# haoyu94/RoITr

Hardware: AMD Instinct MI355X
Metric: point-cloud pairs/s (higher is better)
Workload: dtype f32

## Files before the change

include/roitr_engine.h:

```cpp
#ifndef ROITR_ENGINE_H
#define ROITR_ENGINE_H

#include <stddef.h>

#ifdef __cplusplus
extern "C" {
#endif

#ifndef ROITR_POINTOPS_H
typedef struct ihipStream_t* roitr_stream_t;
#endif

typedef struct RoitrGemm {
    int M, N, K;
    const float* A; const float* A2; int lda; const int* a_idx; int a_limit;
    const float* W; int ldw; const int* w_idx; int w_limit;
    const float* bias; float alpha; int relu;
    float* C; int ldc;
    int batch; long sA, sW, sC, sBias, sAidx, sWidx;
    const int* seg_off; int seg_a0, seg_w0;
    const float* ln_gamma; const float* ln_beta; const float* ln_res; const int* ln_res_idx; const float* ln_post;
    int ln_relu; float ln_eps;
    int bf16;
    const float* A_cat; int lda_cat; int k_cat;
    const float* ip_feat; const int* ip_idx; const float* ip_dist2;
    const int* a_cat_idx;
    const int* batch_live;
    long w_piece;
} RoitrGemm;
#define ROITR_BF16_W 1
#define ROITR_BF16_A 2
#define ROITR_BF16_C 4
#define ROITR_BF16_X3 8
int roitr_gemm(const RoitrGemm* g, roitr_stream_t stream);
int roitr_gemm_bf16_supported(const RoitrGemm* g);
int roitr_f32_to_bf16(long n, const float* src, unsigned short* dst, roitr_stream_t stream);
int roitr_gemm_x3_supported(const RoitrGemm* g);
int roitr_split_bf16x3(long n, const float* src, unsigned short* dst, long piece, roitr_stream_t stream);

int roitr_add_layernorm(int M, int C, const float* x, const float* res, const int* res_idx, const float* gamma,
                        const float* beta, const float* post_add, int relu, float eps, float* out, roitr_stream_t stream);
int roitr_add_layernorm_interp(int M, int C, const float* x, const float* res, const int* res_idx, const float* gamma,
                               const float* beta, int relu, float eps, const float* ip_feat, const int* ip_idx, const float* ip_dist2,
                               float* out, roitr_stream_t stream);
int roitr_l2_normalize(int M, int C, const float* x, float* out, roitr_stream_t stream);
int roitr_transpose(int rows, int cols, const float* in, int ld_in, float* out, int ld_out, roitr_stream_t stream);
int roitr_add_vectors(int n, const float* a, const float* b, float* out, roitr_stream_t stream);
int roitr_interp3_add(int n, int C, const float* feat, const int* idx, const float* dist2, const float* base, float* out,
                      roitr_stream_t stream);
int roitr_segment_mean(int b, int C, const float* x, const int* offset, float* out, roitr_stream_t stream);
int roitr_sinusoid(long rows, int C, const float* vals, const float* div_term, float* out, roitr_stream_t stream);
int roitr_geo_embed(long rows, int C, int angle_k, const float* d_idx, const float* a_idx, const float* div_term,
                    const float* Wd, const float* bd, const float* Wa, const float* ba, float* out, roitr_stream_t stream);
int roitr_split3_bf16(long n, const float* src, unsigned short* dst, roitr_stream_t stream);
int roitr_geo_embed_split(long rows, int C, int angle_k, const float* d_idx, const float* a_idx, const float* div_term,
                          const unsigned short* Wd3, const float* bd, const unsigned short* Wa3, const float* ba, float* out,
                          roitr_stream_t stream);
int roitr_geo_embed_bf16(long rows, int C, int angle_k, const float* d_idx, const float* a_idx, const float* div_term,
                         const unsigned short* Wd, const float* bd, const unsigned short* Wa, const float* ba, float* out,
                         roitr_stream_t stream);
int roitr_geo_embed_bf16_out(long rows, int C, int angle_k, const float* d_idx, const float* a_idx, const float* div_term,
                             const unsigned short* Wd, const float* bd, const unsigned short* Wa, const float* ba,
                             unsigned short* out, roitr_stream_t stream);
size_t roitr_geo_table_floats(int C, int n_int_d, int n_int_a);
int roitr_geo_table_build(int C, const float* div_term, const float* Wd, const float* bd, const float* Wa, const float* ba,
                          float interval, int n_int_d, int n_int_a, float* table, double* fit);
int roitr_geo_embed_table(long rows, int C, int angle_k, const float* d_idx, const float* a_idx, const float* table, float interval,
                          int n_int_d, int n_int_a, const float* div_term, const float* Wd, const float* bd, const float* Wa,
                          const float* ba, void* out, int out_bf16, roitr_stream_t stream);
int roitr_geo_combine(long rows, int C, int k, const float* pd, const float* pa, float* out, roitr_stream_t stream);
int roitr_gather_rows(long rows, int C, const float* in, const int* idx, int limit, float* out, roitr_stream_t stream);
int roitr_compose_idx(int n, const int* outer, const int* inner, int* out, roitr_stream_t stream);
int roitr_calc_ppf(int m, int k, const float* centre_xyz, const float* centre_normals, const float* ref_xyz,
                   const float* ref_normals, const int* group_idx, float* out, roitr_stream_t stream);

typedef struct RoitrLocalAttn {
    int M, K, H, heads;
    const float* q; int ldq;
    const float* k; int ldk;
    const float* v; int ldv;
    const int* group_idx; const float* ppf;
    const float* wvpe; const float* bvpe;
    float scale;
    float* out; int ldo;
    const void* node_order;
    int bf16;
    const float* wpe; const float* bpe;
} RoitrLocalAttn;
int roitr_local_attention(const RoitrLocalAttn* a, roitr_stream_t stream);
int roitr_build_pfold(int H, int heads, const float* wpe, const float* bpe, float* pfold, roitr_stream_t stream);

typedef struct RoitrLocalAttnFold {
    int M, in_dim, H;
    const float* x; int ldx;
    const float* q; int ldq;
    const float* qt;
    const int* group_idx; const float* ppf;
    const float* wpe;
    const float* wvpe; const float* bvpe;
    float scale;
    float* xbar;
    float* vpart;
    const void* node_order;
    int ldqt;
} RoitrLocalAttnFold;
int roitr_local_attention_fold(const RoitrLocalAttnFold* a, roitr_stream_t stream);
int roitr_local_attention_fold_supported(int in_dim, int H, int K);

typedef struct RoitrLocalBlock {
    int M, K, H;
    const float* x; const float* kv; const int* group_idx; const float* ppf;
    const void* node_order;
    const float* wq; const float* bq;
    const float* wpe; const float* bpe; const float* wvpe; const float* bvpe;
    const float* wcat; const float* bcat; const float* norm_w; const float* norm_b;
    const float* wout; const float* bout; const float* bn2_w; const float* bn2_b;
    float scale, eps;
    float* out;
    int kv_bf16;
    const unsigned short* wq_h; const unsigned short* wcat_h; const unsigned short* wout_h;
} RoitrLocalBlock;
int roitr_local_block(const RoitrLocalBlock* a, roitr_stream_t stream);
int roitr_local_block_supported(int H, int K);

typedef struct RoitrLocalTd {
    int M, in_dim, H;
    const float* x; const int* node_idx;
    const int* group_idx; const float* ppf;
    const void* node_order;
    const float* wqqt; const float* bqqt;
    const float* wv; const float* bv;
    const float* wpe; const float* wvpe; const float* bvpe;
    const float* wcat; const float* bcat; const float* norm_w; const float* norm_b;
    const float* wout; const float* bout;
    float scale, eps;
    float* out;
} RoitrLocalTd;
int roitr_local_td(const RoitrLocalTd* a, roitr_stream_t stream);
int roitr_local_td_supported(int in_dim, int H, int K);

typedef struct RoitrLocalFirst {
    int M, K;
    const float* x; const int* group_idx; const float* ppf; const void* node_order;
    const float* head_consts; const float* G; const float* zero_bias;
    const float* norm_w; const float* norm_b; const float* wout; const float* bout;
    float scale, eps;
    float* out;
} RoitrLocalFirst;
int roitr_local_first(const RoitrLocalFirst* a, roitr_stream_t stream);

int roitr_geo_indices(int rows, const float* pts, const int* offset, const int* cloud_of_row, const long* eoff,
                      float sigma_d, float sigma_a, int angle_k, int n_max, float* d_idx, float* a_idx, roitr_stream_t stream);
// ... 189 lines not shown
```

roitr_amd/_lib.py:

```python
import ctypes
import os

_HERE = os.path.dirname(os.path.abspath(__file__))
LIB_PATH = os.path.join(_HERE, "lib", "libroitr_hip.so")
_lib = None


class RoitrError(RuntimeError):
    pass


def lib():
    global _lib
    if _lib is None:
        if not os.path.exists(LIB_PATH):
            raise RoitrError(
                f"{LIB_PATH} is missing: build it with `python -m roitr_amd.build` "
                "(hipcc --offload-arch=gfx950).  roitr_amd has no CPU fallback.")
        import torch
        _lib = ctypes.CDLL(LIB_PATH)
        _lib.roitr_last_error.restype = ctypes.c_char_p
        _lib.roitr_knn_workspace_bytes.restype = ctypes.c_size_t
        _lib.roitr_geo_table_floats.restype = ctypes.c_size_t
        for name in ("roitr_engine_create",):
            if hasattr(_lib, name):
                getattr(_lib, name).restype = ctypes.c_void_p
    return _lib


def check(status, what=""):
    if status != 0:
        raise RoitrError(f"{what} failed with status {status}: {lib().roitr_last_error().decode()}")


def ptr(t):
    if t is None:
        return ctypes.c_void_p(0)
    if not t.is_cuda:
        raise RoitrError("roitr_amd needs ROCm device tensors (no CPU fallback): got a tensor on " + str(t.device))
    return ctypes.c_void_p(t.data_ptr())


def host_ptr(t):
    if t.is_cuda:
        raise RoitrError("host_ptr: expected a CPU tensor")
    return ctypes.c_void_p(t.data_ptr())


def stream_ptr():
    import torch
    return ctypes.c_void_p(torch.cuda.current_stream().cuda_stream)


def c_float(x):
    return ctypes.c_float(float(x))
```

roitr_amd/csrc/geo_table.hip:

```cpp
#include "common.h"
#include <mutex>
#include "prof.h"
#include <cmath>
#include <vector>

namespace {

constexpr int NCOEF = 8, CS = 64;

__device__ __forceinline__ void sincos_cw(float x, float& sn, float& cs)
{
    const float k = rintf(x * 0.63661977236758134f);
    float r = fmaf(-k, 1.57079637050628662109375f, x);
    r = fmaf(-k, -4.37113900018624283e-8f, r);
    r = fmaf(-k, -1.71512449944201e-15f, r);
    const float z = r * r;
    float ps = fmaf(fmaf(-1.9515295891e-4f, z, 8.3321608736e-3f), z, -1.6666654611e-1f);
    ps = fmaf(ps * z, r, r);
    float pc = fmaf(fmaf(2.443315711809948e-5f, z, -1.388731625493765e-3f), z, 4.166664568298827e-2f);
    pc = fmaf(pc * z, z, fmaf(-0.5f, z, 1.0f));
    const int q = (int)k;
    const float s1 = (q & 1) ? pc : ps, c1 = (q & 1) ? ps : pc;
    sn = (q & 2) ? -s1 : s1;
    cs = ((q + 1) & 2) ? -c1 : c1;
}

__device__ __noinline__ float geo_direct(float x, const float* __restrict__ W, const float* __restrict__ bias,
                                         const float* __restrict__ div, int C, int col)
{
    const float* w = W + (size_t)col * C;
    float acc = 0.f;
    for (int i = 0; i < C / 2; ++i) {
        float sn, cs;
        sincos_cw(x * div[i], sn, cs);
        acc = fmaf(sn, w[2 * i], acc);
        acc = fmaf(cs, w[2 * i + 1], acc);
    }
    return acc + bias[col];
}

__device__ __forceinline__ float poly8(const float4* __restrict__ p, float t)
{
    const float4 lo = p[0], hi = p[CS];
    float a = fmaf(hi.w, t, hi.z);
    a = fmaf(a, t, hi.y);
    a = fmaf(a, t, hi.x);
    a = fmaf(a, t, lo.w);
    a = fmaf(a, t, lo.z);
    a = fmaf(a, t, lo.y);
    return fmaf(a, t, lo.x);
}

__device__ __forceinline__ void locate(float x, float inv_h, int n, int base, int& j, float& t)
{
    const float u = x * inv_h;
    const float fl = floorf(u);
    const bool ok = u >= 0.f && fl < (float)n;
    j = ok ? base + (int)fl : -1;
    t = fmaf(2.f, u - fl, -1.f);
}

struct GeoTableArgs {
    long rows;
    int C, nd, na;
    float inv_h;
    const float *d_idx, *a_idx, *table, *div, *Wd, *bd, *Wa, *ba;
    void* out;
};

template <bool OH>
__device__ __forceinline__ void geo_table_body(const GeoTableArgs& g)
{
    extern __shared__ __attribute__((aligned(16))) float tab[];
    const int tid = threadIdx.x, lane = tid & 63, wave = tid >> 6, nwaves = blockDim.x >> 6;
    const int slice = blockIdx.x, nint = g.nd + g.na;
    {
        const float4* src = reinterpret_cast<const float4*>(g.table + (size_t)slice * nint * (NCOEF * CS));
        float4* dst = reinterpret_cast<float4*>(tab);
        for (int i = tid; i < nint * (NCOEF * CS / 4); i += blockDim.x) dst[i] = src[i];
    }
    __syncthreads();
    const int col = slice * CS + lane;
    const float4* tl = reinterpret_cast<const float4*>(tab) + lane;
    const long nchunks = (g.rows + 63) >> 6;
    for (long q = (long)blockIdx.y * nwaves + wave; q < nchunks; q += (long)gridDim.y * nwaves) {
        const long row0 = q << 6, row = row0 + lane;
        float xd = 0.f, xa0 = 0.f, xa1 = 0.f, xa2 = 0.f;
        if (row < g.rows) {
            xd = g.d_idx[row];
            xa0 = g.a_idx[row * 3]; xa1 = g.a_idx[row * 3 + 1]; xa2 = g.a_idx[row * 3 + 2];
        }
        int jd, j0, j1, j2; float td, t0, t1, t2;
        locate(xd, g.inv_h, g.nd, 0, jd, td);
        locate(xa0, g.inv_h, g.na, g.nd, j0, t0);
        locate(xa1, g.inv_h, g.na, g.nd, j1, t1);
        locate(xa2, g.inv_h, g.na, g.nd, j2, t2);
        const int cnt = (int)min(64L, g.rows - row0);
#pragma unroll 2
        for (int e = 0; e < cnt; ++e) {
            const int sjd = __builtin_amdgcn_readlane(jd, e), sj0 = __builtin_amdgcn_readlane(j0, e);
            const int sj1 = __builtin_amdgcn_readlane(j1, e), sj2 = __builtin_amdgcn_readlane(j2, e);
            const float std_ = __uint_as_float(__builtin_amdgcn_readlane(__float_as_uint(td), e));
            const float st0 = __uint_as_float(__builtin_amdgcn_readlane(__float_as_uint(t0), e));
            const float st1 = __uint_as_float(__builtin_amdgcn_readlane(__float_as_uint(t1), e));
            const float st2 = __uint_as_float(__builtin_amdgcn_readlane(__float_as_uint(t2), e));
            float vd, v0, v1, v2;
            if (__builtin_expect((sjd | sj0 | sj1 | sj2) >= 0, 1)) {
                vd = poly8(tl + sjd * (2 * CS), std_);
                v0 = poly8(tl + sj0 * (2 * CS), st0);
                v1 = poly8(tl + sj1 * (2 * CS), st1);
                v2 = poly8(tl + sj2 * (2 * CS), st2);
            } else {
                const float sxd = __uint_as_float(__builtin_amdgcn_readlane(__float_as_uint(xd), e));
                const float sx0 = __uint_as_float(__builtin_amdgcn_readlane(__float_as_uint(xa0), e));
                const float sx1 = __uint_as_float(__builtin_amdgcn_readlane(__float_as_uint(xa1), e));
                const float sx2 = __uint_as_float(__builtin_amdgcn_readlane(__float_as_uint(xa2), e));
                vd = sjd >= 0 ? poly8(tl + sjd * (2 * CS), std_) : geo_direct(sxd, g.Wd, g.bd, g.div, g.C, col);
                v0 = sj0 >= 0 ? poly8(tl + sj0 * (2 * CS), st0) : geo_direct(sx0, g.Wa, g.ba, g.div, g.C, col);
                v1 = sj1 >= 0 ? poly8(tl + sj1 * (2 * CS), st1) : geo_direct(sx1, g.Wa, g.ba, g.div, g.C, col);
                v2 = sj2 >= 0 ? poly8(tl + sj2 * (2 * CS), st2) : geo_direct(sx2, g.Wa, g.ba, g.div, g.C, col);
            }
            const float val = vd + fmaxf(v0, fmaxf(v1, v2));
            const size_t o = (size_t)(row0 + e) * g.C + col;
            if (OH) {
                typedef __bf16 bf16x2_t __attribute__((ext_vector_type(2)));
                typedef float f32x2_t __attribute__((ext_vector_type(2)));
                const float vo = __int_as_float(__builtin_amdgcn_update_dpp(0, __float_as_int(val), 0xB1, 0xf, 0xf, true));
                f32x2_t pr = {val, vo};
                if ((threadIdx.x & 1) == 0)
                    *reinterpret_cast<unsigned*>(reinterpret_cast<unsigned short*>(g.out) + o) = __builtin_bit_cast(unsigned, __builtin_convertvector(pr, bf16x2_t));
            } else reinterpret_cast<float*>(g.out)[o] = val;
        }
    }
}

__global__ __launch_bounds__(1024) void geo_table_kernel(GeoTableArgs g) { geo_table_body<false>(g); }
__global__ __launch_bounds__(1024) void geo_table_bf16o_kernel(GeoTableArgs g) { geo_table_body<true>(g); }

void exact_rows(double x, const std::vector<double>& div, const float* W, const float* b, int C, std::vector<double>& emb, double* out)
{
    for (int i = 0; i < C / 2; ++i) { emb[2 * i] = sin(x * div[i]); emb[2 * i + 1] = cos(x * div[i]); }
    for (int c = 0; c < C; ++c) {
        const float* w = W + (size_t)c * C;
        double s = 0.0;
        for (int k = 0; k < C; ++k) s += (double)w[k] * emb[k];
        out[c] = s + (double)b[c];
    }
}

}

extern "C" size_t roitr_geo_table_floats(int C, int n_int_d, int n_int_a)
{
    return (size_t)(C / CS) * (size_t)(n_int_d + n_int_a) * NCOEF * CS;
}

extern "C" int roitr_geo_table_build(int C, const float* div_term, const float* Wd, const float* bd, const float* Wa, const float* ba,
                                     float interval, int n_int_d, int n_int_a, float* table, double* fit)
{
    if (C % CS || C <= 0 || n_int_d < 1 || n_int_a < 1 || !(interval > 0.f)) return ROITR_ERR_ARG;
    {
        int ex; if (frexpf(interval, &ex) != 0.5f) return ROITR_ERR_ARG;
    }
    const double h = interval;
    std::vector<double> div(C / 2), emb(C);
    for (int i = 0; i < C / 2; ++i) div[i] = (double)div_term[i];
    double node[NCOEF], tm[NCOEF][NCOEF] = {};
    for (int k = 0; k < NCOEF; ++k) node[k] = cos(M_PI * (2 * k + 1) / (2.0 * NCOEF));
    tm[0][0] = 1.0; tm[1][1] = 1.0;
    for (int m = 2; m < NCOEF; ++m)
        for (int p = 0; p < NCOEF; ++p) tm[m][p] = (p > 0 ? 2.0 * tm[m - 1][p - 1] : 0.0) - tm[m - 2][p];
    constexpr int NPROBE = 64;
    std::vector<double> f((size_t)NCOEF * C), mono((size_t)NCOEF * C), ref(C);
    std::vector<double> err_c[2] = {std::vector<double>(C, 0.0), std::vector<double>(C, 0.0)};
    std::vector<double> amp_c[2] = {std::vector<double>(C, 0.0), std::vector<double>(C, 0.0)};
    const int nint = n_int_d + n_int_a;
    for (int q = 0; q < 6; ++q) fit[q] = 0.0;
    for (int J = 0; J < nint; ++J) {
        const bool dist = J < n_int_d;
        const float* W = dist ? Wd : Wa; const float* b = dist ? bd : ba;
        const double x0 = ((dist ? J : J - n_int_d) + 0.5) * h;
        for (int k = 0; k < NCOEF; ++k) exact_rows(x0 + 0.5 * h * node[k], div, W, b, C, emb, &f[(size_t)k * C]);
        for (int c = 0; c < C; ++c) {
            double a[NCOEF];
            for (int m = 0; m < NCOEF; ++m) {
                double s = 0.0;
                for (int k = 0; k < NCOEF; ++k) s += f[(size_t)k * C + c] * cos(M_PI * m * (2 * k + 1) / (2.0 * NCOEF));
                a[m] = s * (m == 0 ? 1.0 : 2.0) / NCOEF;
            }
            for (int p = 0; p < NCOEF; ++p) {
                double s = 0.0;
                for (int m = p; m < NCOEF; ++m) s += a[m] * tm[m][p];
                mono[(size_t)p * C + c] = s;
                table[((((size_t)(c / CS) * nint + J) * 2 + p / 4) * CS + (c % CS)) * 4 + (p % 4)] = (float)s;
            }
        }
        for (int pi = 0; pi < NPROBE; ++pi) {
            const double t = -1.0 + 2.0 * pi / (double)(NPROBE - 1);
            exact_rows(x0 + 0.5 * h * t, div, W, b, C, emb, ref.data());
            for (int c = 0; c < C; ++c) {
                double v = mono[(size_t)(NCOEF - 1) * C + c];
                for (int p = NCOEF - 2; p >= 0; --p) v = v * t + mono[(size_t)p * C + c];
                double& e = fit[dist ? 0 : 2]; double& amp = fit[dist ? 1 : 3];
                const double d = fabs(v - ref[c]);
                e = fmax(e, d); amp = fmax(amp, fabs(ref[c]));
                err_c[dist ? 0 : 1][c] = fmax(err_c[dist ? 0 : 1][c], d);
                amp_c[dist ? 0 : 1][c] = fmax(amp_c[dist ? 0 : 1][c], fabs(ref[c]));
            }
        }
    }
    for (int q = 0; q < 2; ++q) {
        const double floor_ = fit[q ? 3 : 1] / 1024.0;
        for (int c = 0; c < C; ++c) {
            const double a_ = fmax(amp_c[q][c], floor_);
            if (a_ > 0.0) fit[4 + q] = fmax(fit[4 + q], err_c[q][c] / a_);
        }
    }
    return ROITR_OK;
}

extern "C" int roitr_geo_embed_table(long rows, int C, int angle_k, const float* d_idx, const float* a_idx, const float* table,
                                     float interval, int n_int_d, int n_int_a, const float* div_term, const float* Wd, const float* bd,
                                     const float* Wa, const float* ba, void* out, int out_bf16, hipStream_t stream)
{
    if (rows <= 0) return ROITR_OK;
    if (C % CS || angle_k != 3 || n_int_d < 1 || n_int_a < 1) return ROITR_ERR_UNSUPPORTED;
    const size_t lds = (size_t)(n_int_d + n_int_a) * NCOEF * CS * sizeof(float);
    if (lds > 160 * 1024) return ROITR_ERR_UNSUPPORTED;
    {
        static std::mutex mu;
        static size_t granted[64] = {0};
        int dev = 0;
        ROITR_HIP(hipGetDevice(&dev));
        std::lock_guard<std::mutex> lk(mu);
        if (dev < 0 || dev >= 64 || lds > granted[dev]) {
            ROITR_HIP(hipFuncSetAttribute(reinterpret_cast<const void*>(geo_table_kernel), hipFuncAttributeMaxDynamicSharedMemorySize, (int)lds));
            ROITR_HIP(hipFuncSetAttribute(reinterpret_cast<const void*>(geo_table_bf16o_kernel), hipFuncAttributeMaxDynamicSharedMemorySize, (int)lds));
            if (dev >= 0 && dev < 64) granted[dev] = lds;
        }
    }
    GeoTableArgs g;
    g.rows = rows; g.C = C; g.nd = n_int_d; g.na = n_int_a; g.inv_h = 1.0f / interval;
    g.d_idx = d_idx; g.a_idx = a_idx; g.table = table; g.div = div_term; g.Wd = Wd; g.bd = bd; g.Wa = Wa; g.ba = ba; g.out = out;
    const int slices = C / CS;
    const int per_cu = lds <= 80 * 1024 ? 2 : 1;
    static const int cus = [] { hipDeviceProp_t p; int d = 0; (void)hipGetDevice(&d); return hipGetDeviceProperties(&p, d) == hipSuccess ? p.multiProcessorCount : 256; }();
    const int threads = per_cu == 2 ? 512 : 1024;
    const long nchunks = (rows + 63) / 64;
    long gy = ((long)cus * per_cu + slices - 1) / slices;
    gy = std::max(1L, std::min(gy, (nchunks + threads / 64 - 1) / (threads / 64)));
    roitr_prof_begin(ROITR_PROF_GEO_TABLE, (double)rows * C * (out_bf16 ? 2.0 : 4.0) + (double)rows * 16.0 * slices, stream);
    roitr_prof_note(ROITR_PROF_GEO_ALGO, 2.0 * rows * (1.0 + angle_k) * (double)C * C);
    if (out_bf16) geo_table_bf16o_kernel<<<dim3(slices, (unsigned)gy), threads, lds, stream>>>(g);
    else geo_table_kernel<<<dim3(slices, (unsigned)gy), threads, lds, stream>>>(g);
    roitr_prof_end(ROITR_PROF_GEO_TABLE, stream);
    ROITR_LAUNCH_CHECK();
    return ROITR_OK;
}
```

roitr_amd/ops.py:

```python
import torch

from . import _lib as L


def _i32c(t):
    return t.to(torch.int32).contiguous()


def calc_ppf(points, point_normals, ref_points, ref_normals, group_idx):
    m, k = group_idx.shape
    out = torch.empty((m, k, 4), dtype=torch.float32, device=points.device)
    grp = _i32c(group_idx)
    L.check(L.lib().roitr_calc_ppf(m, k, L.ptr(points.contiguous()), L.ptr(point_normals.contiguous()),
                                   L.ptr(ref_points.contiguous()), L.ptr(ref_normals.contiguous()), L.ptr(grp), L.ptr(out),
                                   L.stream_ptr()), "calc_ppf")
    return out


def calc_ppf_gpu(points, point_normals, patches, patch_normals):
    m, k, _ = patches.shape
    grp = torch.arange(m * k, dtype=torch.int32, device=points.device).view(m, k)
    return calc_ppf(points, point_normals, patches.reshape(-1, 3), patch_normals.reshape(-1, 3), grp)


# ... 169 lines not shown
              L.ptr(out), N, 1, 0, 0, 0, 0, 0, 0, L.ptr(None), 0, 0)
    g.bf16 = flags
    keep = []
    _k_cat(g, x, x_cat, keep, x_cat_idx, addend)
    g.ldw = weight.shape[1]
    if x3:
        _x3(g, weight, keep)
    L.check(L.lib().roitr_gemm(ctypes.byref(g), L.stream_ptr()), "gemm")
    return out


def linear_layernorm(x, weight, bias, gamma, beta, res=None, res_idx=None, post=None, relu=False, eps=1e-5, bf16=False, out_bf16=False,
                     x_cat=None, interp=None, x_cat_idx=None, addend=None, x3=False):
    x, weight, flags = _bf16_flags(bf16, x, weight, out_bf16)
    M, K = x.shape
    N = weight.shape[0]
    out = torch.empty((M, N), dtype=torch.bfloat16 if flags & BF16_C else torch.float32, device=x.device)
    c = lambda t, dt=torch.float32: None if t is None else t.contiguous().to(dt)
    b, gm, bt, rs, ri, po = c(bias), c(gamma), c(beta), c(res), c(res_idx, torch.int32), c(post)
    g = _Gemm(M, N, K, L.ptr(x), L.ptr(None), K, L.ptr(None), 0, L.ptr(weight), K, L.ptr(None), 0, L.ptr(b), 1.0, 0,
              L.ptr(out), N, 1, 0, 0, 0, 0, 0, 0, L.ptr(None), 0, 0, L.ptr(gm), L.ptr(bt), L.ptr(rs), L.ptr(ri), L.ptr(po), int(relu), float(eps))
    g.bf16 = flags
    keep = []
    _k_cat(g, x, x_cat, keep, x_cat_idx, addend)
    g.ldw = weight.shape[1]
    if interp is not None:
        keep += [c(interp[0]), c(interp[1], torch.int32), c(interp[2])]
        g.ip_feat, g.ip_idx, g.ip_dist2 = L.ptr(keep[-3]), L.ptr(keep[-2]), L.ptr(keep[-1])
    if x3:
        _x3(g, weight, keep)
    L.check(L.lib().roitr_gemm(ctypes.byref(g), L.stream_ptr()), "gemm+layernorm")
    return out


def add_layernorm_interp(x, gamma, beta, feat, idx, dist2, res=None, res_idx=None, relu=False, eps=1e-5):
    c = lambda t, dt=torch.float32: None if t is None else t.contiguous().to(dt)
    x, gm, bt, rs, ri, ft, ix, d2 = c(x), c(gamma), c(beta), c(res), c(res_idx, torch.int32), c(feat), c(idx, torch.int32), c(dist2)
    M, C = x.shape
    out = torch.empty_like(x)
    L.check(L.lib().roitr_add_layernorm_interp(M, C, L.ptr(x), L.ptr(rs), L.ptr(ri), L.ptr(gm), L.ptr(bt), int(relu), ctypes.c_float(eps),
                                               L.ptr(ft), L.ptr(ix), L.ptr(d2), L.ptr(out), L.stream_ptr()), "add_layernorm_interp")
    return out


def adaptive_superpoint_matching(src_feats, tgt_feats, src_masks, tgt_masks, min_num_correspondences=128, similarity_threshold=0.75):
    dev = src_feats.device
    na, nb = src_feats.shape[0], tgt_feats.shape[0]
    lib = L.lib()
    lib.roitr_coarse_scratch_floats.restype = ctypes.c_size_t
    xy = linear(src_feats, tgt_feats)
    feats = torch.cat([tgt_feats, src_feats], 0).contiguous().float()
    masks = torch.cat([tgt_masks, src_masks], 0).to(torch.int32).contiguous()
    off = torch.tensor([nb, nb + na], dtype=torch.int32, device=dev)
    stride = lib.roitr_coarse_scratch_floats(na, nb)
    scratch = torch.empty(stride, dtype=torch.float32, device=dev)
    cap = na * nb
    ia = torch.zeros(cap, dtype=torch.int32, device=dev)
    ib = torch.zeros(cap, dtype=torch.int32, device=dev)
    sc = torch.zeros(cap, dtype=torch.float32, device=dev)
    nc = torch.zeros(1, dtype=torch.int32, device=dev)
    a = _Coarse(1, feats.shape[1], cap, 0, na, nb, L.ptr(feats), L.ptr(off), L.ptr(masks), L.ptr(scratch), stride, L.ptr(ia), L.ptr(ib),
                L.ptr(sc), L.ptr(nc), L.ptr(xy), 0, nb)
    L.check(lib.roitr_adaptive_matching(ctypes.byref(a), int(min_num_correspondences), ctypes.c_float(similarity_threshold),
                                        L.stream_ptr()), "adaptive_matching")
    n = int(nc.item())
    return ia[:n].long(), ib[:n].long(), sc[:n]


def geo_table_build(div_term, w_d, b_d, w_a, b_a, interval=2.0, d_range=48.0, a_range=12.0):
    import math
    C = int(w_d.shape[0])
    nd, na = int(math.ceil(d_range / interval)), int(math.floor(a_range / interval)) + 1
    lib = L.lib()
    h = lambda t: t.detach().float().cpu().contiguous()
    div_h, wd_h, bd_h, wa_h, ba_h = map(h, (div_term, w_d, b_d, w_a, b_a))
    table = torch.empty(int(lib.roitr_geo_table_floats(C, nd, na)), dtype=torch.float32)
    fit = (ctypes.c_double * 6)()
    hp = L.host_ptr
    L.check(lib.roitr_geo_table_build(C, hp(div_h), hp(wd_h), hp(bd_h), hp(wa_h), hp(ba_h), L.c_float(interval), nd, na,
                                      hp(table), fit), "geo_table_build")
    return table.to(w_d.device), nd, na, list(fit)


def geo_embed_table(d_idx, a_idx, table, interval, n_int_d, n_int_a, div_term, w_d, b_d, w_a, b_a, out_bf16=False):
    rows, k = int(a_idx.shape[0]), int(a_idx.shape[1])
    C = int(w_d.shape[0])
    f = lambda t: t.contiguous().float()
    d_idx, a_idx, table, div_term, w_d, b_d, w_a, b_a = map(f, (d_idx, a_idx, table, div_term, w_d, b_d, w_a, b_a))
    out = torch.empty((rows, C), dtype=torch.bfloat16 if out_bf16 else torch.float32, device=d_idx.device)
    L.check(L.lib().roitr_geo_embed_table(ctypes.c_long(rows), C, k, L.ptr(d_idx), L.ptr(a_idx), L.ptr(table), L.c_float(interval),
                                          int(n_int_d), int(n_int_a), L.ptr(div_term), L.ptr(w_d), L.ptr(b_d), L.ptr(w_a), L.ptr(b_a),
                                          L.ptr(out), 1 if out_bf16 else 0, L.stream_ptr()), "geo_embed_table")
    return out


def geo_embed(d_idx, a_idx, div_term, w_d, b_d, w_a, b_a, split=False, bf16=False):
    rows, k = int(a_idx.shape[0]), int(a_idx.shape[1])
    C = int(w_d.shape[0])
    f = lambda t: t.contiguous().float()
    d_idx, a_idx, div_term, w_d, b_d, w_a, b_a = map(f, (d_idx, a_idx, div_term, w_d, b_d, w_a, b_a))
    out = torch.empty((rows, C), dtype=torch.float32, device=d_idx.device)
    lib = L.lib()
    if bf16:
        wdh, wah = w_d.to(torch.bfloat16).contiguous(), w_a.to(torch.bfloat16).contiguous()
        L.check(lib.roitr_geo_embed_bf16(ctypes.c_long(rows), C, k, L.ptr(d_idx), L.ptr(a_idx), L.ptr(div_term), L.ptr(wdh), L.ptr(b_d),
                                         L.ptr(wah), L.ptr(b_a), L.ptr(out), L.stream_ptr()), "geo_embed_bf16")
        return out
    if split:
        wd3 = torch.empty((3, C, C), dtype=torch.int16, device=out.device)
        wa3 = torch.empty((3, C, C), dtype=torch.int16, device=out.device)
        L.check(lib.roitr_split3_bf16(ctypes.c_long(C * C), L.ptr(w_d), L.ptr(wd3), L.stream_ptr()), "split3")
        L.check(lib.roitr_split3_bf16(ctypes.c_long(C * C), L.ptr(w_a), L.ptr(wa3), L.stream_ptr()), "split3")
        L.check(lib.roitr_geo_embed_split(ctypes.c_long(rows), C, k, L.ptr(d_idx), L.ptr(a_idx), L.ptr(div_term), L.ptr(wd3), L.ptr(b_d),
                                          L.ptr(wa3), L.ptr(b_a), L.ptr(out), L.stream_ptr()), "geo_embed_split")
    else:
        L.check(lib.roitr_geo_embed(ctypes.c_long(rows), C, k, L.ptr(d_idx), L.ptr(a_idx), L.ptr(div_term), L.ptr(w_d), L.ptr(b_d),
                                    L.ptr(w_a), L.ptr(b_a), L.ptr(out), L.stream_ptr()), "geo_embed")
    return out


class _LocalAttnFold(ctypes.Structure):
    _fields_ = [("M", ctypes.c_int), ("in_dim", ctypes.c_int), ("H", ctypes.c_int),
                ("x", ctypes.c_void_p), ("ldx", ctypes.c_int), ("q", ctypes.c_void_p), ("ldq", ctypes.c_int),
                ("qt", ctypes.c_void_p), ("group_idx", ctypes.c_void_p), ("ppf", ctypes.c_void_p),
                ("wpe", ctypes.c_void_p), ("wvpe", ctypes.c_void_p), ("bvpe", ctypes.c_void_p), ("scale", ctypes.c_float),
                ("xbar", ctypes.c_void_p), ("vpart", ctypes.c_void_p), ("node_order", ctypes.c_void_p), ("ldqt", ctypes.c_int)]


def local_attention_fold(x, q, qt, group_idx, ppf, wpe, wvpe, bvpe, node_order=None, packed=False):
    f = lambda t: t.contiguous().float()
    x, q, qt, ppf, wpe, wvpe, bvpe = f(x), f(q), f(qt), f(ppf), f(wpe), f(wvpe), f(bvpe)
    both = torch.cat([q, qt.reshape(q.shape[0], -1)], 1).contiguous() if packed else None
    group_idx = _i32c(group_idx)
    M, H, I = int(q.shape[0]), int(q.shape[1]), int(x.shape[1])
    if int(group_idx.shape[1]) != 16:
        raise L.RoitrError("local_attention_fold: 16 neighbours per node")
    xbar = torch.empty((M, 4, I), dtype=torch.float32, device=x.device)
    vpart = torch.empty((M, H), dtype=torch.float32, device=x.device)
    a = _LocalAttnFold()
    a.M, a.in_dim, a.H = M, I, H
    a.x, a.ldx, a.q, a.ldq, a.qt = L.ptr(x), I, L.ptr(q), H, L.ptr(qt)
    if packed:
        a.q, a.ldq, a.ldqt = L.ptr(both), H + 4 * I, H + 4 * I
        a.qt = ctypes.c_void_p(both.data_ptr() + 4 * H)
    a.group_idx, a.ppf, a.wpe, a.wvpe, a.bvpe = L.ptr(group_idx), L.ptr(ppf), L.ptr(wpe), L.ptr(wvpe), L.ptr(bvpe)
    a.scale, a.xbar, a.vpart = 1.0 / float(H // 4) ** 0.5, L.ptr(xbar), L.ptr(vpart)
    no = f(node_order) if node_order is not None else None
    a.node_order = L.ptr(no)
    L.check(L.lib().roitr_local_attention_fold(ctypes.byref(a), L.stream_ptr()), "local_attention_fold")
    return xbar, vpart


class _LocalTd(ctypes.Structure):
    _fields_ = [("M", ctypes.c_int), ("in_dim", ctypes.c_int), ("H", ctypes.c_int),
                ("x", ctypes.c_void_p), ("node_idx", ctypes.c_void_p), ("group_idx", ctypes.c_void_p), ("ppf", ctypes.c_void_p),
                ("node_order", ctypes.c_void_p), ("wqqt", ctypes.c_void_p), ("bqqt", ctypes.c_void_p), ("wv", ctypes.c_void_p),
                ("bv", ctypes.c_void_p), ("wpe", ctypes.c_void_p), ("wvpe", ctypes.c_void_p), ("bvpe", ctypes.c_void_p),
                ("wcat", ctypes.c_void_p), ("bcat", ctypes.c_void_p), ("norm_w", ctypes.c_void_p), ("norm_b", ctypes.c_void_p),
                ("wout", ctypes.c_void_p), ("bout", ctypes.c_void_p), ("scale", ctypes.c_float), ("eps", ctypes.c_float), ("out", ctypes.c_void_p)]


def local_td(x, node_idx, group_idx, ppf, w, node_order=None):
    f = lambda t: t.contiguous().float()
    x, ppf = f(x), f(ppf)
    node_idx, group_idx = _i32c(node_idx), _i32c(group_idx)
    w = {k: f(v) for k, v in w.items()}
    M, I, H = int(node_idx.shape[0]), int(x.shape[1]), int(w["wout"].shape[0])
    if int(group_idx.shape[1]) != 16 or not L.lib().roitr_local_td_supported(I, H, 16):
        raise L.RoitrError("local_td: in_dim 64, H 128, 16 neighbours per node")
    out = torch.empty((M, H), dtype=torch.float32, device=x.device)
    a = _LocalTd()
    a.M, a.in_dim, a.H = M, I, H
    a.x, a.node_idx, a.group_idx, a.ppf = L.ptr(x), L.ptr(node_idx), L.ptr(group_idx), L.ptr(ppf)
    no = f(node_order) if node_order is not None else None
    a.node_order = L.ptr(no)
# ... 109 lines not shown
```

roitr_amd/riga.py:

```python
import ctypes
import math
import time

import numpy as np
import torch
import torch.nn as nn

from . import _lib as L


def _linear(prefix, out, inp):
    return [(prefix + ".weight", (out, inp), "param"), (prefix + ".bias", (out,), "param")]


def _norm(prefix, c):
    return [(prefix + ".weight", (c,), "param"), (prefix + ".bias", (c,), "param")]


def _local_transformer(prefix, inp, hidden, out):
    ent = [(prefix + ".embedding.embedding.div_term", (hidden // 2,), "buffer")]
    ent += _linear(prefix + ".embedding.proj", hidden, 4)
    ent += _linear(prefix + ".in_proj", hidden, inp)
    for n in ("proj_q", "proj_k", "proj_v", "proj_p", "proj_vp"):
        ent += _linear(prefix + ".transformer.attention." + n, hidden, hidden)
# ... 182 lines not shown
        cfg.fine_conf = self.fine_conf
        cfg.n_geo_layers = len(self.architecture)
        for i, a in enumerate(self.architecture):
            cfg.geo_is_cross[i] = 0 if a == "self" else 1
        cfg.matching_radius = self.matching_radius
        cfg.adaptive_coarse = 0 if self.factor == 1 else 1
        cfg.occlusion_radius = 0.0375
        cfg.operand_dtype = {"f32": 0, "bf16": 1, "f32x3": 2}[self.operand_dtype]
        lib.roitr_engine_create.restype = ctypes.c_void_p
        h = lib.roitr_engine_create(ctypes.byref(cfg))
        if not h:
            raise L.RoitrError("roitr_engine_create failed")
        return ctypes.c_void_p(h)

    def sync_engine(self):
        lib = L.lib()
        if self._engine is None:
            self._engine = self._make_engine()
        for k, v in self.state_dict(keep_vars=True).items():
            if not v.is_cuda:
                raise L.RoitrError(f"parameter {k} is not on a ROCm device: call model.cuda() (no CPU fallback)")
            if v.dtype != torch.float32 or not v.is_contiguous():
                raise L.RoitrError(f"parameter {k} must be contiguous float32")
            L.check(lib.roitr_engine_set_param(self._engine, k.encode(), L.ptr(v), ctypes.c_long(v.numel())), "set_param")
        L.check(lib.roitr_engine_finalize(self._engine, L.stream_ptr()), "engine_finalize")
        self._holders = list(self.modules())
        self._engine_sig = self._weights_signature()

    def _weights_signature(self):
        return [(t.data_ptr(), t._version) for m in self._holders for d in (m._parameters, m._buffers) for t in d.values() if t is not None]

    def _ensure_engine(self):
        if self._engine is None or (not self.weights_frozen and self._weights_signature() != self._engine_sig):
            self.sync_engine()

    def set_tap(self, name, tensor):
        self._ensure_engine()
        self._taps = getattr(self, "_taps", {})
        self._taps[name] = tensor
        L.lib().roitr_engine_set_tap(self._engine, name.encode(), L.ptr(tensor))

    def set_inject(self, name, tensor):
        self._ensure_engine()
        self._injects = getattr(self, "_injects", {})
        self._injects[name] = tensor
        L.lib().roitr_engine_set_inject(self._engine, name.encode(), L.ptr(tensor))

    PROF_CLASSES = {"fps_kernel": 0, "knn_query_kernel": 1, "grid_build_kernel": 2, "knn_replay_kernel": 3, "phase.geometry": 4,
                    "phase.encoder": 5, "phase.global_transformer": 6, "phase.decoder": 7, "phase.matching": 8,
                    "phase.forward": 9, "ot_kernel": 10, "local_attn_kernel": 11, "gemm_kernel.mfma_roofed": 12, "mha_kernel": 13,
                    "geo_embed_kernel": 14, "geo_table_kernel": 15, "geo_embed_reference_flops": 16, "local_block_kernel": 17,
                    "gemm_kernel.hbm_roofed": 18}

    @staticmethod
    def profile_reset(enable=True):
        lib = L.lib()
        lib.roitr_prof_enable(1 if enable else 0)
        lib.roitr_prof_reset()

    @classmethod
    def profile_read(cls, kernels_only=True):
        lib = L.lib()
        out = {}
        for name, cid in cls.PROF_CLASSES.items():
            ms, n, by = ctypes.c_double(0), ctypes.c_long(0), ctypes.c_double(0)
            lib.roitr_prof_read(cid, ctypes.byref(ms), ctypes.byref(n), ctypes.byref(by))
            aux = ctypes.c_double(0)
            lib.roitr_prof_read_aux(cid, ctypes.byref(aux))
            if n.value and (not kernels_only or not name.startswith("phase.")):
                out[name] = {"ms": ms.value, "launches": n.value, "bytes": by.value, "aux": aux.value}
        parts = [out[k] for k in ("gemm_kernel.mfma_roofed", "gemm_kernel.hbm_roofed") if k in out]
        if parts:
            out["gemm_kernel"] = {f: sum(p[f] for p in parts) for f in ("ms", "launches", "bytes", "aux")}
        lib.roitr_prof_enable(0)
        return out

    def geo_table_info(self):
        self._ensure_engine()
        info = (ctypes.c_double * 9)()
        if not L.lib().roitr_engine_geo_table_info(self._engine, info):
            return None
        keys = ("interval", "n_int_d", "n_int_a", "fit_d", "amp_d", "fit_a", "amp_a", "rel_d", "rel_a")
        out = dict(zip(keys, list(info)))
        out["lds_bytes"] = int((out["n_int_d"] + out["n_int_a"]) * 8 * 64 * 4)
        return out

    def __del__(self):
        try:
            if self._engine is not None:
                L.lib().roitr_engine_destroy(self._engine)
        except Exception:
            pass

    @staticmethod
    def level_sizes(n):
        return [n, n // 4, n // 4 // 4, n // 4 // 4 // 4]

    def forward_batch(self, pairs, want_gt=True, graph=False):
        return self.finish_batch(self.launch_batch(pairs, want_gt, graph=graph))

    GRAPH_RING = 3

    @staticmethod
    def _have_gt(pairs, want_gt):
        if not want_gt:
            return False
        flags = [p.get("rot") is not None and p.get("trans") is not None for p in pairs]
        if any(flags) and not all(flags):
            missing = [i for i, f in enumerate(flags) if not f]
            raise L.RoitrError(f"pairs {missing} of this batch have no rot/trans while others do: pass want_gt=False or give "
                               "every pair its ground-truth transform")
        return all(flags)

    def _patch_geometry(self, B, n4, patch_slots=None):
        if self.factor == 1:
            P = self.num_est_coarse_corr
            return P, B * P
        n4max = max(n4)
        P = n4max * n4max
        slots = B * min(P, self.patch_slots_per_pair) if patch_slots is None else int(patch_slots)
        return P, max(1, min(slots, B * P))

    def _alloc_outputs(self, dev, B, T, n4, have_gt, patch_slots=None):
        f32, i32 = torch.float32, torch.int32
        T4, n4max = sum(n4), max(n4)
        C = 256 * self.factor
        P, S = self._patch_geometry(B, n4, patch_slots)
        Lm = self.point_per_patch
        cap = S * Lm * self.fine_topk * (1 if self.fine_mutual else 2)
        z = lambda shape, dt=f32: torch.empty(shape, dtype=dt, device=dev)
        out = dict(node_xyz=z((T4, 3)), node_feats=z((T4, C)), point_feats=z((T, C)), node_masks=z((T4,), i32),
                   node_knn_idx=z((T4, Lm), i32), node_knn_mask=z((T4, Lm), i32), tgt_corr=z((B, P), i32), src_corr=z((B, P), i32),
                   corr_scores=z((B, P)), n_corr=z((B,), i32), tgt_knn_pts=z((S, Lm, 3)), src_knn_pts=z((S, Lm, 3)),
                   tgt_knn_masks=z((S, Lm), i32), src_knn_masks=z((S, Lm), i32), matching_scores=z((S, Lm + 1, Lm + 1)),
                   out_tgt_pts=z((cap, 3)), out_src_pts=z((cap, 3)), out_scores=z((cap,)), out_patch=z((cap,), i32),
                   fine_offsets=z((S,), i32), n_out=z((1,), i32), pair_starts=z((B + 1,), i32))
        if have_gt:
            out.update(gt_node_occ=z((T4,)), gt_corr_idx=z((B, n4max * n4max, 2), i32), gt_corr_overlaps=z((B, n4max * n4max)),
                       gt_corr_count=z((B,), i32))
        return out, P, S

    def launch_batch(self, pairs, want_gt=True, graph=False, inputs_resident=None, patch_slots=None):
        self._ensure_engine()
        if graph:
            return self._launch_graph(pairs, want_gt)
        t_host = time.perf_counter()
        dev = pairs[0]["src_pcd"].device
        B = len(pairs)
        f32 = torch.float32
        n_src = [int(p["src_raw_pcd"].shape[0]) for p in pairs]
        n_tgt = [int(p["tgt_pcd"].shape[0]) for p in pairs]
        n_all = n_src + n_tgt
        T = sum(n_all)
        have_gt = self._have_gt(pairs, want_gt)
        cat = lambda ks, kt: torch.cat([p[ks].to(f32) for p in pairs] + [p[kt].to(f32) for p in pairs], 0).contiguous()

        def pack_inputs():
            rot = trans = None
            if have_gt:
                rot = torch.stack([p["rot"].reshape(3, 3).to(f32) for p in pairs]).contiguous()
                trans = torch.stack([p["trans"].reshape(3).to(f32) for p in pairs]).contiguous()
            return (cat("src_raw_pcd", "tgt_pcd"), cat("src_pcd", "tgt_pcd"), cat("src_normals", "tgt_normals"), cat("src_feats", "tgt_feats"),
                    rot, trans)

        ready = None
        if self.inputs_resident if inputs_resident is None else inputs_resident:
            if self._pack_stream is None:
# ... 179 lines not shown
```

Before: 6401.

## Hold angle polynomial table in registers instead of LDS for geo embedding

When there are at most 13 angle intervals, each lane now loads its angle polynomial coefficients into registers and picks one with a binary select tree instead of reading them from LDS. Only the distance table stays in LDS, which shrinks LDS use and may allow two blocks per CU. The block size drops to 768 threads to leave room for the extra registers. The select tree adds branch and VALU work per lookup, and register pressure could reduce occupancy.

```diff
diff --git a/include/roitr_engine.h b/include/roitr_engine.h
--- a/include/roitr_engine.h
+++ b/include/roitr_engine.h
@@ -68,6 +68,10 @@
 int roitr_geo_embed_table(long rows, int C, int angle_k, const float* d_idx, const float* a_idx, const float* table, float interval,
                           int n_int_d, int n_int_a, const float* div_term, const float* Wd, const float* bd, const float* Wa,
                           const float* ba, void* out, int out_bf16, roitr_stream_t stream);
+int roitr_geo_embed_table_form(long rows, int C, int angle_k, const float* d_idx, const float* a_idx, const float* table, float interval,
+                               int n_int_d, int n_int_a, const float* div_term, const float* Wd, const float* bd, const float* Wa,
+                               const float* ba, void* out, int out_bf16, int form, roitr_stream_t stream);
+size_t roitr_geo_table_lds_bytes(int n_int_d, int n_int_a);
 int roitr_geo_combine(long rows, int C, int k, const float* pd, const float* pa, float* out, roitr_stream_t stream);
 int roitr_gather_rows(long rows, int C, const float* in, const int* idx, int limit, float* out, roitr_stream_t stream);
 int roitr_compose_idx(int n, const int* outer, const int* inner, int* out, roitr_stream_t stream);
diff --git a/roitr_amd/_lib.py b/roitr_amd/_lib.py
--- a/roitr_amd/_lib.py
+++ b/roitr_amd/_lib.py
@@ -22,6 +22,7 @@
         _lib.roitr_last_error.restype = ctypes.c_char_p
         _lib.roitr_knn_workspace_bytes.restype = ctypes.c_size_t
         _lib.roitr_geo_table_floats.restype = ctypes.c_size_t
+        _lib.roitr_geo_table_lds_bytes.restype = ctypes.c_size_t
         for name in ("roitr_engine_create",):
             if hasattr(_lib, name):
                 getattr(_lib, name).restype = ctypes.c_void_p
diff --git a/roitr_amd/csrc/geo_table.hip b/roitr_amd/csrc/geo_table.hip
--- a/roitr_amd/csrc/geo_table.hip
+++ b/roitr_amd/csrc/geo_table.hip
@@ -39,9 +39,8 @@
     return acc + bias[col];
 }
 
-__device__ __forceinline__ float poly8(const float4* __restrict__ p, float t)
-{
-    const float4 lo = p[0], hi = p[CS];
+__device__ __forceinline__ float horner8(const float4 lo, const float4 hi, float t)
+{
     float a = fmaf(hi.w, t, hi.z);
     a = fmaf(a, t, hi.y);
     a = fmaf(a, t, hi.x);
@@ -51,6 +50,27 @@
     return fmaf(a, t, lo.x);
 }
 
+__device__ __forceinline__ float poly8(const float4* __restrict__ p, float t) { return horner8(p[0], p[CS], t); }
+
+constexpr int NA_REG = 13;
+
+template <int LO, int HI>
+__device__ __forceinline__ float poly8_sel(const float4 (&lo)[NA_REG], const float4 (&hi)[NA_REG], int j, float t)
+{
+    if constexpr (LO == HI) {
+        float r = horner8(lo[LO], hi[LO], t);
+        asm volatile("" : "+v"(r));
+        return r;
+    } else {
+        constexpr int MID = (LO + HI) / 2;
+        return j <= MID ? poly8_sel<LO, MID>(lo, hi, j, t) : poly8_sel<MID + 1, HI>(lo, hi, j, t);
+    }
+}
+__device__ __forceinline__ float poly8_reg(const float4 (&lo)[NA_REG], const float4 (&hi)[NA_REG], int j, float t)
+{
+    return poly8_sel<0, NA_REG - 1>(lo, hi, j, t);
+}
+
 __device__ __forceinline__ void locate(float x, float inv_h, int n, int base, int& j, float& t)
 {
     const float u = x * inv_h;
@@ -68,20 +88,30 @@
     void* out;
 };
 
-template <bool OH>
+template <bool OH, bool RG>
 __device__ __forceinline__ void geo_table_body(const GeoTableArgs& g)
 {
     extern __shared__ __attribute__((aligned(16))) float tab[];
     const int tid = threadIdx.x, lane = tid & 63, wave = tid >> 6, nwaves = blockDim.x >> 6;
     const int slice = blockIdx.x, nint = g.nd + g.na;
+    const float4* src = reinterpret_cast<const float4*>(g.table + (size_t)slice * nint * (NCOEF * CS));
     {
-        const float4* src = reinterpret_cast<const float4*>(g.table + (size_t)slice * nint * (NCOEF * CS));
         float4* dst = reinterpret_cast<float4*>(tab);
-        for (int i = tid; i < nint * (NCOEF * CS / 4); i += blockDim.x) dst[i] = src[i];
+        for (int i = tid; i < (RG ? g.nd : nint) * (NCOEF * CS / 4); i += blockDim.x) dst[i] = src[i];
+    }
+    float4 alo[NA_REG], ahi[NA_REG];
+    if (RG) {
+#pragma unroll
+        for (int j = 0; j < NA_REG; ++j) {
+            const int jj = g.nd + min(j, g.na - 1);
+            alo[j] = src[jj * (2 * CS) + lane];
+            ahi[j] = src[jj * (2 * CS) + CS + lane];
+        }
     }
     __syncthreads();
-    const int col = slice * CS + lane;
+    const int col = slice * CS + lane, abase = RG ? 0 : g.nd;
     const float4* tl = reinterpret_cast<const float4*>(tab) + lane;
+    auto angle = [&](int j, float t) { return RG ? poly8_reg(alo, ahi, j, t) : poly8(tl + j * (2 * CS), t); };
     const long nchunks = (g.rows + 63) >> 6;
     for (long q = (long)blockIdx.y * nwaves + wave; q < nchunks; q += (long)gridDim.y * nwaves) {
         const long row0 = q << 6, row = row0 + lane;
@@ -92,9 +122,9 @@
         }
         int jd, j0, j1, j2; float td, t0, t1, t2;
         locate(xd, g.inv_h, g.nd, 0, jd, td);
-        locate(xa0, g.inv_h, g.na, g.nd, j0, t0);
-        locate(xa1, g.inv_h, g.na, g.nd, j1, t1);
-        locate(xa2, g.inv_h, g.na, g.nd, j2, t2);
+        locate(xa0, g.inv_h, g.na, abase, j0, t0);
+        locate(xa1, g.inv_h, g.na, abase, j1, t1);
+        locate(xa2, g.inv_h, g.na, abase, j2, t2);
         const int cnt = (int)min(64L, g.rows - row0);
 #pragma unroll 2
         for (int e = 0; e < cnt; ++e) {
@@ -107,18 +137,18 @@
             float vd, v0, v1, v2;
             if (__builtin_expect((sjd | sj0 | sj1 | sj2) >= 0, 1)) {
                 vd = poly8(tl + sjd * (2 * CS), std_);
-                v0 = poly8(tl + sj0 * (2 * CS), st0);
-                v1 = poly8(tl + sj1 * (2 * CS), st1);
-                v2 = poly8(tl + sj2 * (2 * CS), st2);
+                v0 = angle(sj0, st0);
+                v1 = angle(sj1, st1);
+                v2 = angle(sj2, st2);
             } else {
                 const float sxd = __uint_as_float(__builtin_amdgcn_readlane(__float_as_uint(xd), e));
                 const float sx0 = __uint_as_float(__builtin_amdgcn_readlane(__float_as_uint(xa0), e));
                 const float sx1 = __uint_as_float(__builtin_amdgcn_readlane(__float_as_uint(xa1), e));
                 const float sx2 = __uint_as_float(__builtin_amdgcn_readlane(__float_as_uint(xa2), e));
                 vd = sjd >= 0 ? poly8(tl + sjd * (2 * CS), std_) : geo_direct(sxd, g.Wd, g.bd, g.div, g.C, col);
-                v0 = sj0 >= 0 ? poly8(tl + sj0 * (2 * CS), st0) : geo_direct(sx0, g.Wa, g.ba, g.div, g.C, col);
-                v1 = sj1 >= 0 ? poly8(tl + sj1 * (2 * CS), st1) : geo_direct(sx1, g.Wa, g.ba, g.div, g.C, col);
-                v2 = sj2 >= 0 ? poly8(tl + sj2 * (2 * CS), st2) : geo_direct(sx2, g.Wa, g.ba, g.div, g.C, col);
+                v0 = sj0 >= 0 ? angle(sj0, st0) : geo_direct(sx0, g.Wa, g.ba, g.div, g.C, col);
+                v1 = sj1 >= 0 ? angle(sj1, st1) : geo_direct(sx1, g.Wa, g.ba, g.div, g.C, col);
+                v2 = sj2 >= 0 ? angle(sj2, st2) : geo_direct(sx2, g.Wa, g.ba, g.div, g.C, col);
             }
             const float val = vd + fmaxf(v0, fmaxf(v1, v2));
             const size_t o = (size_t)(row0 + e) * g.C + col;
@@ -134,8 +164,11 @@
     }
 }
 
-__global__ __launch_bounds__(1024) void geo_table_kernel(GeoTableArgs g) { geo_table_body<false>(g); }
-__global__ __launch_bounds__(1024) void geo_table_bf16o_kernel(GeoTableArgs g) { geo_table_body<true>(g); }
+constexpr int REG_THREADS = 768;
+__global__ __launch_bounds__(REG_THREADS) void geo_table_kernel(GeoTableArgs g) { geo_table_body<false, true>(g); }
+__global__ __launch_bounds__(REG_THREADS) void geo_table_bf16o_kernel(GeoTableArgs g) { geo_table_body<true, true>(g); }
+__global__ __launch_bounds__(1024) void geo_table_lds_kernel(GeoTableArgs g) { geo_table_body<false, false>(g); }
+__global__ __launch_bounds__(1024) void geo_table_lds_bf16o_kernel(GeoTableArgs g) { geo_table_body<true, false>(g); }
 
 void exact_rows(double x, const std::vector<double>& div, const float* W, const float* b, int C, std::vector<double>& emb, double* out)
 {
@@ -219,24 +252,46 @@
     return ROITR_OK;
 }
 
-extern "C" int roitr_geo_embed_table(long rows, int C, int angle_k, const float* d_idx, const float* a_idx, const float* table,
-                                     float interval, int n_int_d, int n_int_a, const float* div_term, const float* Wd, const float* bd,
-                                     const float* Wa, const float* ba, void* out, int out_bf16, hipStream_t stream)
+namespace {
+
+int geo_table_form(int form, int n_int_a) { return form ? form : (n_int_a <= NA_REG ? 2 : 1); }
+
+size_t geo_table_lds(int form, int n_int_d, int n_int_a)
+{
+    return (size_t)(form == 2 ? n_int_d : n_int_d + n_int_a) * NCOEF * CS * sizeof(float);
+}
+
+}
+
+extern "C" size_t roitr_geo_table_lds_bytes(int n_int_d, int n_int_a)
+{
+    return geo_table_lds(geo_table_form(0, n_int_a), n_int_d, n_int_a);
+}
+
+extern "C" int roitr_geo_embed_table_form(long rows, int C, int angle_k, const float* d_idx, const float* a_idx, const float* table,
+                                          float interval, int n_int_d, int n_int_a, const float* div_term, const float* Wd,
+                                          const float* bd, const float* Wa, const float* ba, void* out, int out_bf16, int form,
+                                          hipStream_t stream)
 {
     if (rows <= 0) return ROITR_OK;
-    if (C % CS || angle_k != 3 || n_int_d < 1 || n_int_a < 1) return ROITR_ERR_UNSUPPORTED;
-    const size_t lds = (size_t)(n_int_d + n_int_a) * NCOEF * CS * sizeof(float);
+    if (C % CS || angle_k != 3 || n_int_d < 1 || n_int_a < 1 || form < 0 || form > 2) return ROITR_ERR_UNSUPPORTED;
+    form = geo_table_form(form, n_int_a);
+    if (form == 2 && n_int_a > NA_REG) return ROITR_ERR_UNSUPPORTED;
+    const bool rg = form == 2;
+    const size_t lds = geo_table_lds(form, n_int_d, n_int_a);
     if (lds > 160 * 1024) return ROITR_ERR_UNSUPPORTED;
+    const void* kern = rg ? (out_bf16 ? (const void*)geo_table_bf16o_kernel : (const void*)geo_table_kernel)
+                          : (out_bf16 ? (const void*)geo_table_lds_bf16o_kernel : (const void*)geo_table_lds_kernel);
     {
         static std::mutex mu;
-        static size_t granted[64] = {0};
+        static size_t granted[4][64] = {{0}};
         int dev = 0;
         ROITR_HIP(hipGetDevice(&dev));
+        const int ki = (rg ? 2 : 0) + (out_bf16 ? 1 : 0);
         std::lock_guard<std::mutex> lk(mu);
-        if (dev < 0 || dev >= 64 || lds > granted[dev]) {
-            ROITR_HIP(hipFuncSetAttribute(reinterpret_cast<const void*>(geo_table_kernel), hipFuncAttributeMaxDynamicSharedMemorySize, (int)lds));
-            ROITR_HIP(hipFuncSetAttribute(reinterpret_cast<const void*>(geo_table_bf16o_kernel), hipFuncAttributeMaxDynamicSharedMemorySize, (int)lds));
-            if (dev >= 0 && dev < 64) granted[dev] = lds;
+        if (dev < 0 || dev >= 64 || lds > granted[ki][dev]) {
+            ROITR_HIP(hipFuncSetAttribute(kern, hipFuncAttributeMaxDynamicSharedMemorySize, (int)lds));
+            if (dev >= 0 && dev < 64) granted[ki][dev] = lds;
         }
     }
     GeoTableArgs g;
@@ -245,15 +300,29 @@
     const int slices = C / CS;
     const int per_cu = lds <= 80 * 1024 ? 2 : 1;
     static const int cus = [] { hipDeviceProp_t p; int d = 0; (void)hipGetDevice(&d); return hipGetDeviceProperties(&p, d) == hipSuccess ? p.multiProcessorCount : 256; }();
-    const int threads = per_cu == 2 ? 512 : 1024;
+    const int threads = rg ? REG_THREADS / per_cu : (per_cu == 2 ? 512 : 1024);
     const long nchunks = (rows + 63) / 64;
     long gy = ((long)cus * per_cu + slices - 1) / slices;
     gy = std::max(1L, std::min(gy, (nchunks + threads / 64 - 1) / (threads / 64)));
     roitr_prof_begin(ROITR_PROF_GEO_TABLE, (double)rows * C * (out_bf16 ? 2.0 : 4.0) + (double)rows * 16.0 * slices, stream);
     roitr_prof_note(ROITR_PROF_GEO_ALGO, 2.0 * rows * (1.0 + angle_k) * (double)C * C);
-    if (out_bf16) geo_table_bf16o_kernel<<<dim3(slices, (unsigned)gy), threads, lds, stream>>>(g);
-    else geo_table_kernel<<<dim3(slices, (unsigned)gy), threads, lds, stream>>>(g);
+    const dim3 grid(slices, (unsigned)gy);
+    if (rg) {
+        if (out_bf16) geo_table_bf16o_kernel<<<grid, threads, lds, stream>>>(g);
+        else geo_table_kernel<<<grid, threads, lds, stream>>>(g);
+    } else {
+        if (out_bf16) geo_table_lds_bf16o_kernel<<<grid, threads, lds, stream>>>(g);
+        else geo_table_lds_kernel<<<grid, threads, lds, stream>>>(g);
+    }
     roitr_prof_end(ROITR_PROF_GEO_TABLE, stream);
     ROITR_LAUNCH_CHECK();
     return ROITR_OK;
 }
+
+extern "C" int roitr_geo_embed_table(long rows, int C, int angle_k, const float* d_idx, const float* a_idx, const float* table,
+                                     float interval, int n_int_d, int n_int_a, const float* div_term, const float* Wd, const float* bd,
+                                     const float* Wa, const float* ba, void* out, int out_bf16, hipStream_t stream)
+{
+    return roitr_geo_embed_table_form(rows, C, angle_k, d_idx, a_idx, table, interval, n_int_d, n_int_a, div_term, Wd, bd, Wa, ba, out,
+                                      out_bf16, 0, stream);
+}
diff --git a/roitr_amd/ops.py b/roitr_amd/ops.py
--- a/roitr_amd/ops.py
+++ b/roitr_amd/ops.py
@@ -275,15 +275,15 @@
     return table.to(w_d.device), nd, na, list(fit)
 
 
-def geo_embed_table(d_idx, a_idx, table, interval, n_int_d, n_int_a, div_term, w_d, b_d, w_a, b_a, out_bf16=False):
+def geo_embed_table(d_idx, a_idx, table, interval, n_int_d, n_int_a, div_term, w_d, b_d, w_a, b_a, out_bf16=False, form=0):
     rows, k = int(a_idx.shape[0]), int(a_idx.shape[1])
     C = int(w_d.shape[0])
     f = lambda t: t.contiguous().float()
     d_idx, a_idx, table, div_term, w_d, b_d, w_a, b_a = map(f, (d_idx, a_idx, table, div_term, w_d, b_d, w_a, b_a))
     out = torch.empty((rows, C), dtype=torch.bfloat16 if out_bf16 else torch.float32, device=d_idx.device)
-    L.check(L.lib().roitr_geo_embed_table(ctypes.c_long(rows), C, k, L.ptr(d_idx), L.ptr(a_idx), L.ptr(table), L.c_float(interval),
-                                          int(n_int_d), int(n_int_a), L.ptr(div_term), L.ptr(w_d), L.ptr(b_d), L.ptr(w_a), L.ptr(b_a),
-                                          L.ptr(out), 1 if out_bf16 else 0, L.stream_ptr()), "geo_embed_table")
+    L.check(L.lib().roitr_geo_embed_table_form(ctypes.c_long(rows), C, k, L.ptr(d_idx), L.ptr(a_idx), L.ptr(table), L.c_float(interval),
+                                               int(n_int_d), int(n_int_a), L.ptr(div_term), L.ptr(w_d), L.ptr(b_d), L.ptr(w_a), L.ptr(b_a),
+                                               L.ptr(out), 1 if out_bf16 else 0, int(form), L.stream_ptr()), "geo_embed_table")
     return out
 
 
diff --git a/roitr_amd/riga.py b/roitr_amd/riga.py
--- a/roitr_amd/riga.py
+++ b/roitr_amd/riga.py
@@ -288,7 +288,7 @@
             return None
         keys = ("interval", "n_int_d", "n_int_a", "fit_d", "amp_d", "fit_a", "amp_a", "rel_d", "rel_a")
         out = dict(zip(keys, list(info)))
-        out["lds_bytes"] = int((out["n_int_d"] + out["n_int_a"]) * 8 * 64 * 4)
+        out["lds_bytes"] = int(L.lib().roitr_geo_table_lds_bytes(int(out["n_int_d"]), int(out["n_int_a"])))
         return out
 
     def __del__(self):
```

New measurement: 6278. 1.9% lower.
